# mvrl/RANGE

Measured on AMD Instinct MI355X. Metric: geo-embeddings/sec (10k-query batch, range_db_large), higher is better.
Workload: dtype f32

## Files before the change

range_amd/csrc/forward_host.h:

```cpp
#pragma once

struct ModelParams { float tau_sem, tau_geo, beta; };

static int model_params(const range_ctx* c, int32_t model, float beta, ModelParams& m) {
    if (model != RANGE_MODEL_RANGE && model != RANGE_MODEL_RANGE_PLUS)
        return fail(RANGE_ERR_INVALID, "unknown model %d", model);
    m.tau_sem = model == RANGE_MODEL_RANGE ? 15.0f : 12.0f;
    m.tau_geo = model == RANGE_MODEL_RANGE ? 0.0f : 40.0f;
    if (c->tau_sem_set > 0.f) m.tau_sem = c->tau_sem_set;
    if (c->tau_geo_set > 0.f && model == RANGE_MODEL_RANGE_PLUS) m.tau_geo = c->tau_geo_set;
    m.beta = model == RANGE_MODEL_RANGE ? 1.0f : beta;
    if (!(m.beta >= 0.f && m.beta <= 1.f)) return fail(RANGE_ERR_INVALID, "beta must be in [0,1]");
    return RANGE_OK;
}

static int forward_head(const range_ctx* c, const double* lonlat, const double* out, int32_t model, float beta, ModelParams& m) {
    if (!c || !lonlat || !out) return fail(RANGE_ERR_INVALID, "null argument");
    return model_params(c, model, beta, m);
}

static int forward_small(range_ctx* c, int64_t B, const ModelParams& m, double* out, hipStream_t s) {
    SmallArgs a{};
    int rc = softmax_scales(c, B, m.tau_sem, m.tau_geo, RANGE_MAX_TAU, a.k_sem, a.k_geo);
    if (rc) return rc;
    const SmallPlan p = plan_forward_small(c->n_cu, c->bank.n_rows, B, PLAN_CONSTS);
    HIP_TRY(c->pass.ws_small_o.ensure(p.o_floats));
    HIP_TRY(c->pass.ws_small_z.ensure(p.z_floats));
    a.keys = c->bank.d_keys.p;
    a.xyz4 = c->bank.d_xyz4.p;
    a.values = c->bank.d_values.p;
    a.ehat = c->pass.ws_ehat32.p;
    a.xq = c->pass.ws_xq.p;
    a.osum = c->pass.ws_small_o.p;
    a.zsum = c->pass.ws_small_z.p;
    a.B = B;
    a.n_valid = c->bank.n_rows;
    a.n_blocks = p.n_blocks;
    const bool geo = m.tau_geo > 0.f;
    static void (*const small_kernels[2][2])(SmallArgs) = {{attend_small_kernel<true, 2>, attend_small_kernel<true, 1>},
                                                          {attend_small_kernel<false, 2>, attend_small_kernel<false, 1>}};
    {
        ProfScope ps(c, RANGE_PROF_ATTEND, s);
        if (int lrc = launch(small_kernels[!geo][p.nq == 1], dim3((unsigned)p.n_wg), dim3(256), as_lds_bytes(p.nq), s, a)) return lrc;
    }
    rc = launch(small_finalize_kernel, dim3((unsigned)B, 8), dim3(1024), 0, s, c->pass.ws_small_o.p, c->pass.ws_small_z.p,
                p.n_wg, p.qcap, geo ? 1 : 0, geo ? m.beta : 1.0f, c->pass.ws_ehat64.p, out);
    if (rc) return rc;
    c->pass.last_qtiles = 1;
    c->pass.last_splits = p.n_wg;
    return RANGE_OK;
}

static int scan_workspace(range_ctx* c, int64_t B, const ModelParams& m, bool* kept, range_stream_t stream) {
    const int rc = range_scan_stats(c, c->pass.ws_ehat32.p, c->pass.ws_xq.p, B, m.tau_sem, m.tau_geo, c->pass.ws_stats.p, 0,
                                    nullptr, nullptr, 1, stream);
    *kept = c->kept.kept_B == B;
    return rc;
}

static int attend_workspace(range_ctx* c, int64_t p0, int64_t p1, const ModelParams& m, bool kept, SlabMap* map,
                            range_stream_t stream) {
    return attend_impl(c, c->pass.ws_ehat32.p + p0 * 256, c->pass.ws_xq.p + p0 * 4, p1 - p0, m.tau_sem, m.tau_geo, m.beta,
                       c->pass.ws_stats.p + p0 * 4, nullptr, map, kept ? p0 : -1, stream);
}

static int forward_chunked(range_ctx* c, int64_t B, const ModelParams& m, const FwdChunkPlan& plan, double* out,
                           range_stream_t stream, bool* chunked) {
    *chunked = false;
    ENTER_DEVICE(c);
    hipStream_t s = (hipStream_t)stream;
    const size_t n_chunks = plan.tiles.size();
    if (!c->ovl.aux_stream) {
        HIP_TRY(hipStreamCreateWithFlags(&c->ovl.aux_stream, hipStreamNonBlocking));
    }
    while (c->ovl.events.size() < n_chunks) {
        hipEvent_t e = nullptr;
        HIP_TRY(hipEventCreateWithFlags(&e, hipEventDisableTiming));
        c->ovl.events.push_back(e);
    }
    int64_t most_tiles = 0;
    for (int t : plan.tiles) most_tiles = std::max<int64_t>(most_tiles, t);
    HIP_TRY(c->pass.ws_stats_parts.ensure((size_t)plan.p1_splits * B * 4));
    HIP_TRY(c->pass.ws_slabs.ensure((size_t)plan.p2_splits * std::min<int64_t>(B, most_tiles * QTILE) * VAL_DIM));
    const float* ehat = c->pass.ws_ehat32.p;
    const float* xq = c->pass.ws_xq.p;
    float* stats = c->pass.ws_stats.p;
    std::vector<int64_t> cuts{0};
    for (int t : plan.tiles) cuts.push_back(std::min<int64_t>(B, cuts.back() + (int64_t)t * QTILE));
    if (int rc = scan_stats_impl(c, ehat, xq, cuts[1], m.tau_sem, m.tau_geo, stats, 0, nullptr, nullptr, 1, 0, B,
                                 plan.p1_splits, stream))
        return rc;
    if (c->kept.kept_B != cuts[1]) return RANGE_OK;
    *chunked = true;
    HIP_TRY(hipEventRecord(c->ovl.events[0], s));
    HIP_TRY(hipStreamWaitEvent(c->ovl.aux_stream, c->ovl.events[0], 0));
    size_t recorded = 0;
    auto joined = [&](int rc) {
        (void)hipStreamWaitEvent(s, c->ovl.events[recorded], 0);
        return rc;
    };
    for (size_t i = 1; i < n_chunks; ++i) {
        const int64_t q0 = cuts[i], nq = cuts[i + 1] - q0;
        if (int rc = scan_stats_impl(c, ehat + q0 * KEY_DIM, xq + q0 * 4, nq, m.tau_sem, m.tau_geo, stats + q0 * 4, 0, nullptr, nullptr,
                                     1, q0, B, plan.p1_splits, (range_stream_t)c->ovl.aux_stream, true,
                                     (size_t)plan.p1_splits * q0 * 4))
            return joined(rc);
        HIP_TRY(hipEventRecord(c->ovl.events[i], c->ovl.aux_stream));
        recorded = i;
    }
    for (size_t i = 0; i < n_chunks; ++i) {
        const int64_t q0 = cuts[i], nq = cuts[i + 1] - q0;
        if (i > 0) HIP_TRY(hipStreamWaitEvent(s, c->ovl.events[i], 0));
        SlabMap map{};
        if (int rc = attend_impl(c, ehat + q0 * KEY_DIM, xq + q0 * 4, nq, m.tau_sem, m.tau_geo, m.beta, stats + q0 * 4, nullptr, &map, q0,
                                 stream, nullptr, 0, plan.p2_splits))
            return joined(rc);
        HIP_TRY(launch_finalize(c->pass.ws_slabs.p, map, c->pass.ws_ehat64.p + q0 * KEY_DIM, nq, 0, nq, out + q0 * RANGE_OUT_DIM, s));
    }
    c->pass.last_qtiles = (int)((B + QTILE - 1) / QTILE);
    c->pass.last_splits = plan.p2_splits;
    return RANGE_OK;
}

extern "C" {

int range_forward(range_ctx* c, const double* lonlat, int64_t B, int32_t model, float beta,
                  double* out, range_stream_t stream) {
    ModelParams m;
    if (int rc = forward_head(c, lonlat, out, model, beta, m)) return rc;
    c->pass.ws_queries = 0;
    if (int rc = encode_to_workspace(c, lonlat, B, nullptr, stream)) return rc;
    if (plan_temperatures(m.tau_sem, m.tau_geo, B, c->sw.small_forward).one_pass) {
        c->pass.ws_queries = B;
        ENTER_DEVICE(c);
        return forward_small(c, B, m, out, (hipStream_t)stream);
    }
    if (c->sw.allow_keep && c->bank.pv_mode == RANGE_PV_EXACT && c->bank.has_bank &&
        plan_temperatures(m.tau_sem, m.tau_geo, B, false).shift == SHIFT_CONSTANT) {
        const FwdChunkPlan plan = plan_forward_chunks(c->n_cu, plan_pass1(c->n_cu, c->bank.n_rows, B, false, 0, PLAN_CONSTS),
                                                      plan_pass2(c->n_cu, c->bank.n_rows, B, c->sw.p2_streamk, PLAN_CONSTS),
                                                      c->sw.fwd_overlap);
        if (plan.tiles.size() >= 2) {
            bool chunked = false;
            if (int rc = forward_chunked(c, B, m, plan, out, stream, &chunked)) return rc;
            if (chunked) {
                c->pass.ws_queries = B;
                return RANGE_OK;
            }
        }
    }
    bool kept = false;
    SlabMap map{};
    if (int rc = scan_workspace(c, B, m, &kept, stream)) return rc;
    if (int rc = attend_workspace(c, 0, B, m, kept, &map, stream)) return rc;
    c->pass.ws_queries = B;
    ENTER_DEVICE(c);
    HIP_TRY(launch_finalize(c->pass.ws_slabs.p, map, c->pass.ws_ehat64.p, B, 0, B, out, (hipStream_t)stream));
    return RANGE_OK;
}

int range_host_copy(range_ctx* c, void* dst, const void* src, size_t bytes) {
    if (!c || !dst || !src) return fail(RANGE_ERR_INVALID, "null argument");
    if (!c->host.pool) c->host.pool.reset(new HostCopyPool(HostCopyPool::default_threads()));
    c->host.pool->copy(dst, src, bytes);
    return RANGE_OK;
}

int range_forward_host(range_ctx* c, const double* lonlat, int64_t B, int32_t model, float beta,
                       double* out_host, range_stream_t stream) {
    ModelParams m;
    if (int rc0 = forward_head(c, lonlat, out_host, model, beta, m)) return rc0;
    if (B <= 0) return fail(RANGE_ERR_INVALID, "B must be > 0");
    ENTER_DEVICE(c);
    hipStream_t s = (hipStream_t)stream;
    const size_t row_bytes = (size_t)RANGE_OUT_DIM * sizeof(double);
    HIP_TRY(c->host.ws_out64.ensure((size_t)B * RANGE_OUT_DIM));
    if (c->host.h_stage_bytes < (size_t)B * row_bytes) {
        if (c->host.h_stage) (void)hipHostFree(c->host.h_stage);
        c->host.h_stage = nullptr;
        c->host.h_stage_bytes = 0;
        HIP_TRY(hipHostMalloc(&c->host.h_stage, (size_t)B * row_bytes, hipHostMallocDefault));
        c->host.h_stage_bytes = (size_t)B * row_bytes;
    }
    if (!c->host.copy_stream) HIP_TRY(hipStreamCreateWithFlags(&c->host.copy_stream, hipStreamNonBlocking));
    if (!c->host.pool) c->host.pool.reset(new HostCopyPool(HostCopyPool::default_threads()));

    c->pass.ws_queries = 0;
    int rc = encode_to_workspace(c, lonlat, B, nullptr, stream);
    if (rc) return rc;
    c->pass.ws_queries = B;
    if (plan_temperatures(m.tau_sem, m.tau_geo, B, c->sw.small_forward).one_pass) {
        rc = forward_small(c, B, m, c->host.ws_out64.p, s);
        if (rc) return rc;
        HIP_TRY(hipMemcpyAsync(c->host.h_stage, c->host.ws_out64.p, (size_t)B * row_bytes, hipMemcpyDeviceToHost, s));
        HIP_TRY(hipStreamSynchronize(s));
        if (int rc2 = check_async_error(c)) return rc2;
        std::memcpy(out_host, c->host.h_stage, (size_t)B * row_bytes);
        return RANGE_OK;
    }
    bool kept = false;
    rc = scan_workspace(c, B, m, &kept, stream);
    if (rc) return rc;

    std::vector<int64_t> cuts{0, B};
// ... 54 lines not shown
```

range_amd/csrc/host_plan.h:

```cpp
#pragma once
#include <algorithm>
#include <cmath>
#include <cstddef>
#include <cstdint>
#include <vector>

namespace range_host {

inline int choose_splits(int n_qtiles, int n_blocks, int n_cu, int wg_per_cu, int max_splits,
                         double split_cost = 0.002) {
    const double slots = (double)n_cu * wg_per_cu;
    const int cap = std::max(1, std::min(max_splits, n_blocks / 4));
    const int ns_min = std::min(cap, (int)std::ceil(slots / n_qtiles));
    int best = ns_min;
    double best_score = -1e9;
    for (int ns = ns_min; ns <= cap; ++ns) {
        const double total = (double)n_qtiles * ns;
        const double rounds = std::ceil(total / slots);
        double score = total / (rounds * slots);
        if (rounds < 4) score *= 0.85 + 0.0375 * rounds;
        score -= split_cost * (ns - ns_min);
        if (score > best_score) { best_score = score; best = ns; }
        if (ns - ns_min > 64) break;
    }
// ... 284 lines not shown
    size_t part_floats = 0;
    int64_t topk_slots = 0;
    int topk_chunks = 0;
};

inline Pass1Plan plan_pass1(int n_cu, int64_t n_rows, int64_t B, bool topk_scan, int force_splits, const PlanConsts& K) {
    Pass1Plan p;
    p.n_blocks = (int32_t)((n_rows + K.blk - 1) / K.blk);
    p.n_qtiles = (int32_t)((B + K.qtile - 1) / K.qtile);
    const bool few = B <= 4 * K.qtile;
    p.n_splits = choose_splits(p.n_qtiles, p.n_blocks, n_cu, K.p1_wg_per_cu,
                               topk_scan ? (few ? 256 : 16) : (few ? 2048 : 128));
    if (force_splits > 0) p.n_splits = std::max(1, std::min<int>(force_splits, std::max(1, p.n_blocks / 4)));
    p.grid = p.n_splits * p.n_qtiles;
    p.merge_by_wave = p.n_splits > 32;
    p.part_floats = (size_t)p.n_splits * B * 4;
    p.topk_slots = (B + 15) / 16;
    p.topk_chunks = (int)std::max<int64_t>(1, std::min<int64_t>(
        std::min<int64_t>(64, p.n_blocks / 32 > 0 ? p.n_blocks / 32 : 1),
        ((int64_t)16 * n_cu + p.topk_slots - 1) / p.topk_slots));
    return p;
}

struct KeptStatsPlan {
    int n_qtiles = 0, n_blocks = 0, n_splits = 0;
    int grid = 0;
    bool merge_by_wave = false;
    struct Group { int first, count; };
    std::vector<Group> groups;
    size_t part_floats = 0;
    size_t ws_floats = 0;
};

inline ShiftMode kept_pair_shift(float tau_sem, float tau_geo) { return plan_temperatures(tau_sem, tau_geo, 0, false).shift; }

inline KeptStatsPlan plan_kept_stats(int n_cu, int64_t n_rows, int64_t B, int n_pairs, int force_splits, int max_pairs,
                                     const PlanConsts& K) {
    KeptStatsPlan p;
    const Pass1Plan s = plan_pass1(n_cu, n_rows, B, false, force_splits, K);
    p.n_qtiles = s.n_qtiles;
    p.n_blocks = s.n_blocks;
    p.n_splits = s.n_splits;
    p.grid = s.grid;
    p.merge_by_wave = s.merge_by_wave;
    p.part_floats = s.part_floats;
    for (int first = 0; first < n_pairs; first += max_pairs)
        p.groups.push_back({first, std::min(max_pairs, n_pairs - first)});
    p.ws_floats = p.part_floats * (size_t)std::min(max_pairs, std::max(n_pairs, 0));
    return p;
}

struct Pass2Plan {
    int n_qtiles = 0, n_blocks = 0;
    int n_splits = 0;
    bool streamk = false;
    int sk_cols = 1, sk_groups = 0;
    int grid = 0;
    size_t slab_floats = 0;
};

inline Pass2Plan plan_pass2(int n_cu, int64_t n_rows, int64_t B, bool allow_streamk, const PlanConsts& K,
                            int force_splits = 0) {
    Pass2Plan p;
    p.n_blocks = (int32_t)((n_rows + K.blk - 1) / K.blk);
    p.n_qtiles = (int32_t)((B + K.qtile - 1) / K.qtile);
    p.n_splits = choose_splits(p.n_qtiles, p.n_blocks, n_cu, 1,
                               std::max(32, std::min(512, (n_cu + p.n_qtiles - 1) / p.n_qtiles)),
                               std::max(0.001, 140.0 / (double)n_rows));
    if (force_splits > 0) p.n_splits = std::max(1, std::min<int>(force_splits, std::max(1, p.n_blocks / 4)));
    constexpr int P2_STREAMK_ROWS = 50000;
    p.streamk = allow_streamk && n_rows <= P2_STREAMK_ROWS;
    if (p.streamk) {
        constexpr int P2_COL_ROWS = 16384;
        p.sk_cols = (int32_t)std::max<int64_t>(1, std::min<int64_t>((n_rows + P2_COL_ROWS - 1) / P2_COL_ROWS,
                                                                    std::max(1, p.n_blocks / 4)));
        const int64_t Uc = (int64_t)p.n_qtiles * (p.n_blocks / p.sk_cols);
        p.sk_groups = (int32_t)std::max<int64_t>(1, std::min<int64_t>(n_cu, Uc / 4));
        p.slab_floats = (size_t)p.sk_cols * (p.sk_groups + p.n_qtiles) * K.qtile * K.val_dim;
    } else {
        p.slab_floats = (size_t)p.n_splits * B * K.val_dim;
    }
    p.grid = p.streamk ? p.sk_groups : p.n_splits * p.n_qtiles;
    return p;
}

struct FwdChunkPlan {
    std::vector<int> tiles;
    int p1_splits = 0, p2_splits = 0;
};

constexpr int FWD_CHUNK_FILL_PCT = 98;
inline FwdChunkPlan plan_forward_chunks(int n_cu, const Pass1Plan& p1, const Pass2Plan& p2, int overlap) {
    FwdChunkPlan p;
    p.p1_splits = p1.n_splits;
    p.p2_splits = p2.n_splits;
    const int T = p2.n_qtiles, ns = p2.n_splits;
    if (overlap == 0 || p2.streamk || T < 2 || ns < 1 || n_cu < 1) return p;
    if (overlap > 0) {
        for (int t0 = 0; t0 < T && overlap < T; t0 += overlap) p.tiles.push_back(std::min(overlap, T - t0));
        return p;
    }
    const int64_t R = ((int64_t)T * ns + n_cu - 1) / n_cu;
    for (int64_t C = std::min<int64_t>(R, T); C >= 2; --C) {
        std::vector<int> lo((size_t)C), hi((size_t)C);
        int64_t sum_lo = 0, sum_hi = 0;
        bool ok = true;
        for (int64_t i = 0; i < C && ok; ++i) {
            const int64_t r = R / C + (i >= C - R % C ? 1 : 0);
            const int64_t most = r * n_cu / ns;
            const int64_t fill = (FWD_CHUNK_FILL_PCT * r * n_cu + 100 * (int64_t)ns - 1) / (100 * (int64_t)ns);
            const int64_t least = std::max<int64_t>(std::max<int64_t>(fill, (r - 1) * n_cu / ns + 1), 1);
            ok = least <= most;
            lo[(size_t)i] = (int)least;
            hi[(size_t)i] = (int)most;
            sum_lo += least;
            sum_hi += most;
        }
        if (!ok || sum_lo > T || sum_hi < T) continue;
        p.tiles = hi;
        int64_t excess = sum_hi - T;
        for (size_t i = 0; i < p.tiles.size() && excess > 0; ++i) {
            const int64_t d = std::min<int64_t>(excess, hi[i] - lo[i]);
            p.tiles[i] -= (int)d;
            excess -= d;
        }
        return p;
    }
    return p;
}

struct TopkPlan {
    int n_groups = 0, n_blocks = 0;
    bool gemm = false;
    int G = 1;
    int n_wg = 0;
    bool fused = false;
    size_t cand_keys = 0, cand_dmax = 0;
    int key_e2 = 0;
    int n_qblocks = 0, n_splits = 0, grid = 0;
    int tile_stride = 1;
};

inline TopkPlan plan_topk(int n_cu, int64_t n_rows, int64_t B, float key_norm_max, bool topk_gemm, bool bf16,
                          bool topks_fused, bool force_exact, int tg_sample, const PlanConsts& K) {
    TopkPlan p;
    p.n_groups = (int)((B + 15) / 16);
    p.n_blocks = (int)((n_rows + K.blk - 1) / K.blk);
    constexpr int NWV = 4;
    p.G = p.n_groups <= 1 ? 1 : 2;
    p.n_wg = std::max(1, std::min(std::min(n_cu, 256), (p.n_blocks + NWV - 1) / NWV));
    p.fused = topks_fused && B <= p.n_wg;
    p.cand_keys = (size_t)p.n_groups * 16 * p.n_wg * K.topks_wl;
    p.cand_dmax = (size_t)p.n_groups * 16 * p.n_wg;
    (void)std::frexp((double)key_norm_max, &p.key_e2);
    const bool tg_bank_ok = key_norm_max > 0.f && std::isfinite(key_norm_max) && std::abs(14 - p.key_e2) <= 100;
    p.gemm = topk_gemm && bf16 && B > 256 && p.n_blocks >= 64 && !force_exact && B <= 60000 && tg_bank_ok;
    if (p.gemm) {
        p.n_qblocks = (int32_t)((B + K.tg_qblock - 1) / K.tg_qblock);
        p.n_splits = std::max(4, std::min(std::min(K.tg_wg_per_cu * n_cu / p.n_qblocks, p.n_blocks / 8), 64));
        p.grid = p.n_qblocks * p.n_splits;
        p.tile_stride = std::max(1, std::min(tg_sample, p.n_blocks / p.n_splits / 4));
    }
    return p;
}

struct SmallPlan {
// ... 744 lines not shown
```

range_amd/csrc/pass2.h:

```cpp
#pragma once
#include "scan_common.h"

namespace range_hip {

__device__ __forceinline__ unsigned long long stamp() {
    unsigned long long t;
    asm volatile("s_memtime %0\n\ts_waitcnt lgkmcnt(0)" : "=s"(t) :: "memory");
    return t;
}
#define RANGE_WAIT_BARRIER_DIAG(n, vm, bar)                                   \
    do {                                                                      \
        const unsigned long long t0_ = stamp();                               \
        asm volatile("s_waitcnt vmcnt(" #n ") lgkmcnt(0)" ::: "memory");      \
        const unsigned long long t1_ = stamp();                               \
        asm volatile("s_barrier" ::: "memory");                               \
        const unsigned long long t2_ = stamp();                               \
        vm += t1_ - t0_; bar += t2_ - t1_;                                    \
    } while (0)
#define RANGE_WB(n, vm, bar)                                                  \
    do { if (DIAG) RANGE_WAIT_BARRIER_DIAG(n, vm, bar); else RANGE_WAIT_BARRIER(n); } while (0)

struct PvCarry {
    f32x4 v0a, v1a, v0b, v1b;
    float w0, w1;
// ... 463 lines not shown
                            const int ii = h / 6;
                            if (ii == 0) {
                                dma_b128(ssrc2, vvoff, sdst);
                            } else if (ii == 1) {
                                dma_b32(xsrc2, (uint32_t)(lane << 2), xdst);
                            } else if (ii < 18) {
                                const int p = ii - 2, hh = p >> 3, row = (p >> 2) & 1, qq = p & 3;
                                if (qq == 0) dma_group_begin(vdst + hh * (VB_BYTES / 2) + row * 4096);
                                dma_b128_q(vsrc1 + (8 * hh + row) * VAL_DIM, vvoff, qq);
                            }
                        }
                    } else if (h >= 150 && h < 206 && (h & 1) == 0) {
                        const int k = (h - 150) >> 1, r = k / 7, op = k % 7;
                        if (op == 0) e1[r] = fmaf(sv[r], a.k_sem, -wc.m1);
                        else if (op == 1) { if (GEO) e2[r] = fmaf(cg[r], a.k_geo, -wc.m2); }
                        else if (op == 2) e1[r] = __builtin_amdgcn_exp2f(e1[r]);
                        else if (op == 3) { if (GEO) e2[r] = __builtin_amdgcn_exp2f(e2[r]); }
                        else if (op == 4) e1[r] = valu_mul(wc.ca, e1[r]);
                        else if (op == 5) { if (GEO) e1[r] = valu_fma(wc.cb, e2[r], e1[r]); }
                        else w_next[r] = e1[r];
                    }
                });
    };

    if (nb > 0) {
        const int valid_last = n_left - (nb - 1) * BLK;
        int t = 0;
        for (; t + 2 <= nb; t += 2) {
            run_block(IntC<0>{}, t, w_a, w_b);
            if (t + 2 == nb && valid_last < BLK) zero_pad_rows(w_b, prow, valid_last);
            run_block(IntC<1>{}, t + 1, w_b, w_a);
        }
        if (t < nb) {
            if (valid_last < BLK) zero_pad_rows(w_a, prow, valid_last);
            run_block(IntC<0>{}, t, w_a, w_b);
        }
        carry_wait_states();
        pv_exec_carry(acc, carry);
    }
    asm volatile("s_waitcnt vmcnt(0)" ::: "memory");

    store_acc_tile(acc, out_tile, qt, wave, lane, a.B);
    }
}


template <int UNROLL>
__device__ __forceinline__ f32x4 sum_parts(const float* parts, const SlabMap& m, int64_t B, int64_t q, int c4) {
    f32x4 s = {0.f, 0.f, 0.f, 0.f};
    for (int col = 0; col < slab_cols(m); ++col) {
        int64_t first4, stride4;
        int n;
        slab_parts(m, B, q, col, first4, stride4, n);
        const f32x4* p4 = reinterpret_cast<const f32x4*>(parts) + first4 + c4;
        if (col == 0) s = p4[0];
#pragma unroll UNROLL
        for (int p = col == 0 ? 1 : 0; p < n; ++p) s += p4[(int64_t)p * stride4];
    }
    return s;
}

__global__ void reduce_parts_kernel(const float* parts, SlabMap m, int64_t B, float* out) {
    const int64_t i = (int64_t)blockIdx.x * blockDim.x + threadIdx.x;
    if (i >= B * (VAL_DIM / 4)) return;
    const int64_t q = i / (VAL_DIM / 4);
    const int c4 = (int)(i - q * (VAL_DIM / 4));
    reinterpret_cast<f32x4*>(out)[i] = sum_parts<4>(parts, m, B, q, c4);
}

__global__ void blend_kernel(const float* G, const float* H, float beta, int64_t n4, float* out) {
    const int64_t i = (int64_t)blockIdx.x * blockDim.x + threadIdx.x;
    if (i >= n4) return;
    const f32x4 g = reinterpret_cast<const f32x4*>(G)[i];
    const f32x4 h = reinterpret_cast<const f32x4*>(H)[i];
    const float a = 1.0f - beta;
    f32x4 o;
#pragma unroll
    for (int k = 0; k < 4; ++k) o[k] = __fadd_rn(__fmul_rn(a, g[k]), __fmul_rn(beta, h[k]));
    reinterpret_cast<f32x4*>(out)[i] = o;
}

__global__ void finalize_kernel(const float* parts, SlabMap m, const double* ehat64, int64_t B,
                                int64_t q0, int64_t nq, double* out) {
    const int64_t i = (int64_t)blockIdx.x * blockDim.x + threadIdx.x;
    if (i >= nq * 320) return;
    const int64_t q = q0 + i / 320;
    const int c = (int)(i % 320);
    double* o = out + q * 1280 + 4 * c;
    if (c < 256) {
        const f32x4 s = sum_parts<8>(parts, m, B, q, c);
        o[0] = (double)s.x; o[1] = (double)s.y; o[2] = (double)s.z; o[3] = (double)s.w;
    } else {
        const double* e = ehat64 + q * 256 + 4 * (c - 256);
        o[0] = e[0]; o[1] = e[1]; o[2] = e[2]; o[3] = e[3];
    }
}

}
```

range_amd/csrc/scan_host.h:

```cpp
#pragma once

static_assert(MAX_TAU_CONSTANT == RANGE_MAX_TAU && MAX_TAU_SHARP == RANGE_MAX_TAU_SHARP, "host_plan.h and range_hip.h disagree");

static int softmax_scales(range_ctx* c, int64_t B, float tau_sem, float tau_geo, float max_tau, float& k_sem, float& k_geo) {
    if (!c->bank.has_bank) return fail(RANGE_ERR_STATE, "bank not set (range_set_bank)");
    if (!c->bank.has_values)
        return fail(RANGE_ERR_STATE, "keys-only bank (range_set_keys): only range_topk_stream runs on it");
    if (B <= 0) return fail(RANGE_ERR_INVALID, "B must be > 0");
    if (!plan_temperatures(tau_sem, tau_geo, B, false).valid)
        return fail(RANGE_ERR_INVALID, "temperatures must be finite, > 0 and at most %g (tau_sem %g, tau_geo %g; tau_geo <= 0: "
                    "no geographic head): beyond that the softmax is an argmax to float32 precision",
                    (double)RANGE_MAX_TAU_SHARP, (double)tau_sem, (double)tau_geo);
    if (!(c->bank.key_norm_max <= 1.001f))
        return fail(RANGE_ERR_INVALID, "bank keys are not L2-normalised or not finite (largest row norm %.4f): the softmax of "
                    "range_scan_stats / range_attend needs unit keys, as range/range.py:85-89 prepares them "
                    "(range_topk_stream accepts any norm)", (double)c->bank.key_norm_max);
    if (tau_geo > 0.f && !(c->bank.xyz_norm_max <= 1.001f))
        return fail(RANGE_ERR_INVALID, "bank locations are not unit vectors or not finite (largest row norm %.4f): the geographic "
                    "softmax needs them as range/utils/utils.py:11-16 computes them", (double)c->bank.xyz_norm_max);
    if (tau_sem > max_tau || tau_geo > max_tau)
        return fail(RANGE_ERR_INVALID, "internal: temperatures above %g reached a constant-shift kernel", (double)max_tau);
    const double LOG2E = 1.4426950408889634;
    k_sem = (float)(tau_sem * LOG2E);
    k_geo = tau_geo > 0.f ? (float)(tau_geo * LOG2E) : 0.f;
    return RANGE_OK;
}

static int fill_scan_args(range_ctx* c, ScanArgs& a, const float* ehat32, const float* xq, int64_t B,
                          float tau_sem, float tau_geo) {
    if (int rc = softmax_scales(c, B, tau_sem, tau_geo, RANGE_MAX_TAU_SHARP, a.k_sem, a.k_geo)) return rc;
    a.keys = c->bank.d_keys.p;
    a.xyz4 = c->bank.d_xyz4.p;
    a.values = c->bank.d_values.p;
    a.ehat = ehat32;
    a.xq = xq;
    a.B = B;
    a.n_valid = c->bank.n_rows;
    a.beta = 1.f;
    a.sk_cols = 1;
    return RANGE_OK;
}

static int launch_merge_stats(bool by_wave, const float* parts, int32_t n_parts, int64_t B, float* out, hipStream_t s) {
    const int per_wg = by_wave ? 4 : 256;
    return launch(by_wave ? merge_stats_wave_kernel : merge_stats_kernel, dim3((unsigned)((B + per_wg - 1) / per_wg)), dim3(256),
                  0, s, parts, n_parts, B, out);
}

static hipError_t launch_finalize(const float* slabs, const SlabMap& map, const double* ehat64, int64_t B, int64_t q0,
                                  int64_t nq, double* out, hipStream_t s) {
    const int64_t n = nq * 320;
    hipLaunchKernelGGL(finalize_kernel, dim3((unsigned)((n + 255) / 256)), dim3(256), 0, s, slabs, map, ehat64, B, q0, nq, out);
    return hipGetLastError();
}

static int scan_stats_impl(range_ctx* c, const float* ehat32, const float* xq32, int64_t B, float tau_sem,
                           float tau_geo, float* stats, int topk, float* topk_val, int64_t* topk_idx,
                           int32_t keep_logits, int64_t first_query, int64_t total_queries, int32_t force_splits,
                           range_stream_t stream, bool beside = false, size_t parts_offset = 0) {
    if (!c || !ehat32 || !xq32 || !stats) return fail(RANGE_ERR_INVALID, "null argument");
    if (topk < 0 || topk > MAX_TOPK) return fail(RANGE_ERR_INVALID, "topk must be in [0,%d]", MAX_TOPK);
    if (topk > 0 && (!topk_val || !topk_idx)) return fail(RANGE_ERR_INVALID, "topk outputs null");
    if (first_query < 0 || first_query % QTILE != 0)
        return fail(RANGE_ERR_INVALID, "first_query must be a non-negative multiple of %d", QTILE);
    if (B > 0 && first_query + B > total_queries)
        return fail(RANGE_ERR_INVALID, "queries [%lld, %lld) exceed the scan's %lld", (long long)first_query,
                    (long long)(first_query + B), (long long)total_queries);
    if (force_splits < 0) return fail(RANGE_ERR_INVALID, "n_splits must be >= 0");
    ENTER_DEVICE(c);
    ScanArgs a{};
    hipStream_t s = (hipStream_t)stream;
    const bool extends = first_query > 0 && c->kept.kept_B == first_query && c->kept.kept_total == total_queries;
    if (first_query > 0 && !extends) keep_logits = 0;
    if (!extends) c->kept.kept_B = 0;
    bool write_logits = c->sw.allow_keep && (topk > 0 ? B > 0 : keep_logits != 0);
    const int64_t n_qtiles = (total_queries + QTILE - 1) / QTILE, n_blocks = (c->bank.n_rows + BLK - 1) / BLK;
    const size_t need = (size_t)n_qtiles * n_blocks * 1024;
    if (write_logits && extends) {
        if (need > c->kept.ws_logits.n || c->kept.kept_blocks != n_blocks) { write_logits = false; c->kept.kept_B = 0; }
    } else if (write_logits && need > c->kept.ws_logits.n) {
        size_t free_b = 0, total_b = 0;
        HIP_TRY(hipMemGetInfo(&free_b, &total_b));
        if (need * sizeof(float) <= free_b / 2) {
            HIP_TRY(c->kept.ws_logits.ensure(need));
        } else {
            write_logits = false;
            if (!c->kept.warned_no_keep) {
                c->kept.warned_no_keep = true;
                std::fprintf(stderr, "librange_hip: the logits of %lld queries x %lld bank rows (%.1f GB) do not fit in "
                             "half of the free device memory (%.1f GB free): not kept, pass 2 recomputes them\n",
                             (long long)B, (long long)c->bank.n_rows, need * 4e-9, free_b * 1e-9);
            }
        }
    }
    const bool topk_from_kept = topk > 0 && write_logits;
    const bool topk_scan = topk > 0 && !topk_from_kept;
    int rc = fill_scan_args(c, a, ehat32, xq32, B, tau_sem, tau_geo);
    if (rc) return rc;
    const TempRoute route = plan_temperatures(tau_sem, tau_geo, B, c->sw.small_forward);
    if (topk_scan && !route.topk_scan_ok)
        return fail(RANGE_ERR_INVALID, "range_scan_stats(topk > 0) at a temperature above %g needs to keep its logits (this "
                    "context cannot: RANGE_KEEP_LOGITS=0 or not enough free memory): take the top-k from range_topk_stream",
                    (double)RANGE_MAX_TAU);
    const Pass1Plan p = plan_pass1(c->n_cu, c->bank.n_rows, B, topk_scan, force_splits, PLAN_CONSTS);
    a.n_blocks = p.n_blocks;
    a.n_qtiles = p.n_qtiles;
    a.n_splits = p.n_splits;
    if (write_logits) a.logits = c->kept.ws_logits.p;
    a.qt_offset = (int32_t)(first_query / QTILE);
    if (topk_from_kept) {
        HIP_TRY(c->kept.ws_rowmax.ensure(p.part_floats));
        HIP_TRY(c->kept.ws_theta.ensure((size_t)B));
        a.rowmax = c->kept.ws_rowmax.p;
    }
    HIP_TRY(c->pass.ws_stats_parts.ensure(parts_offset + p.part_floats));
    a.out = c->pass.ws_stats_parts.p + parts_offset;
    if (topk_scan) {
        HIP_TRY(c->topk.ws_cand_val.ensure(p.part_floats * MAX_TOPK));
        HIP_TRY(c->topk.ws_cand_idx.ensure(p.part_floats * MAX_TOPK));
        a.cand_val = c->topk.ws_cand_val.p;
        a.cand_idx = c->topk.ws_cand_idx.p;
    }
    const bool geo = tau_geo > 0.f;
    static void (*const scan_kernels[2][2])(ScanArgs) = {{scan_stats_kernel<true, true>, scan_stats_kernel<true, false>},
                                                        {scan_stats_kernel<false, true>, scan_stats_kernel<false, false>}};
    static void (*const sharp_kernels[2])(ScanArgs) = {sharp_scan_stats_kernel<true>, sharp_scan_stats_kernel<false>};
    static void (*const beside_kernels[2])(ScanArgs) = {scan_stats_beside_kernel<true>, scan_stats_beside_kernel<false>};
    if (beside && (topk > 0 || route.shift == SHIFT_RUNNING_MAX))
        return fail(RANGE_ERR_INVALID, "internal: pass 1 beside pass 2 has the constant shift and no top-k");
    {
        ProfScope ps(c, RANGE_PROF_SCAN_STATS, s);
        if (beside) {
            if (int lrc = launch(beside_kernels[!geo], dim3((unsigned)std::min(c->n_cu, p.grid)), dim3(256), BESIDE_LDS_BYTES, s, a)) return lrc;
        } else {
            void (*const kernel)(ScanArgs) = route.shift == SHIFT_RUNNING_MAX ? sharp_kernels[!geo] : scan_kernels[!geo][!topk_scan];
            if (int lrc = launch(kernel, dim3((unsigned)p.grid), dim3(256), SCAN_LDS_BYTES, s, a)) return lrc;
        }
    }
    if (a.logits && keep_logits) {
        c->kept.kept_B = first_query + B;
        c->kept.kept_total = total_queries;
        c->kept.kept_blocks = a.n_blocks;
    }
    rc = launch_merge_stats(p.merge_by_wave, a.out, a.n_splits, B, stats, s);
    if (rc) return rc;
    int n_parts = a.n_splits, per_part = 4 * MAX_TOPK;
    if (topk_from_kept) {
        const int n_chunks = p.topk_chunks;
        HIP_TRY(c->topk.ws_cand_val.ensure((size_t)n_chunks * B * MAX_TOPK));
        HIP_TRY(c->topk.ws_cand_idx.ensure((size_t)n_chunks * B * MAX_TOPK));
        rc = launch(topk_threshold_kernel, dim3((unsigned)((B + 3) / 4)), dim3(256), 0, s,
                    c->kept.ws_rowmax.p, a.n_splits, B, c->kept.ws_theta.p);
        if (rc) return rc;
        rc = launch(topk_from_logits_kernel, dim3((unsigned)((p.topk_slots + 3) / 4), (unsigned)n_chunks),
                    dim3(256), 0, s, c->kept.ws_logits.p, a.n_blocks, B, c->bank.n_rows, n_chunks,
                    c->kept.ws_theta.p, c->topk.ws_cand_val.p, c->topk.ws_cand_idx.p);
        if (rc) return rc;
        n_parts = n_chunks;
        per_part = MAX_TOPK;
    }
    if (topk <= 0) return RANGE_OK;
    return launch(merge_topk_wave_kernel, dim3((unsigned)((B + 3) / 4)), dim3(256), 0, s, c->topk.ws_cand_val.p,
                  c->topk.ws_cand_idx.p, n_parts, B, per_part, topk, c->bank.row_offset, topk_val, topk_idx);
}

static int attend_impl(range_ctx* c, const float* ehat32, const float* xq32, int64_t B, float tau_sem,
                       float tau_geo, float beta, const float* stats_global, float* partial,
                       SlabMap* map_out, int64_t kept_first, range_stream_t stream,
                       unsigned long long* diag_dev = nullptr, int64_t diag_capacity = 0, int32_t force_splits = 0) {
    if (!c || (!ehat32 && kept_first < 0) || !xq32 || !stats_global)
        return fail(RANGE_ERR_INVALID, "null argument");
    if (kept_first >= 0) {
        if (c->kept.kept_B <= 0) return fail(RANGE_ERR_STATE, "no kept logits (range_scan_stats with keep_logits)");
        if (kept_first % QTILE != 0) return fail(RANGE_ERR_INVALID, "first kept query must be a multiple of %d", QTILE);
        if (kept_first + B > c->kept.kept_B)
            return fail(RANGE_ERR_INVALID, "queries [%lld, %lld) exceed the %lld kept", (long long)kept_first,
                        (long long)(kept_first + B), (long long)c->kept.kept_B);
    }
    if (!diag_dev && !(beta >= 0.f && beta <= 1.f)) return fail(RANGE_ERR_INVALID, "beta must be in [0,1]");
    ENTER_DEVICE(c);
    ScanArgs a{};
    int rc = fill_scan_args(c, a, ehat32, xq32, B, tau_sem, tau_geo);
    if (rc) return rc;
    hipStream_t s = (hipStream_t)stream;
    const bool geo = tau_geo > 0.f;
    const bool bf16x3 = kept_first >= 0 && c->bank.pv_mode == RANGE_PV_BF16X3;
    if (bf16x3 && plan_temperatures(tau_sem, tau_geo, B, false).shift == SHIFT_RUNNING_MAX)
        return fail(RANGE_ERR_INVALID, "pv mode bf16x3 is not supported at temperatures above %g", (double)RANGE_MAX_TAU);
    const Pass2Plan p = plan_pass2(c->n_cu, c->bank.n_rows, B, c->sw.p2_streamk && !bf16x3 && !diag_dev, PLAN_CONSTS, force_splits);
    a.n_blocks = p.n_blocks;
    a.n_qtiles = p.n_qtiles;
    a.n_splits = p.n_splits;
    a.sk_cols = p.sk_cols;
    a.sk_groups = p.sk_groups;
    c->pass.last_qtiles = p.n_qtiles;
    c->pass.last_splits = p.streamk ? p.sk_groups : p.n_splits;
    if (diag_dev) {
        if (!geo) return fail(RANGE_ERR_INVALID, "diagnostic build exists for the geo variant only");
        if ((int64_t)p.grid * 4 * 16 > diag_capacity) return fail(RANGE_ERR_INVALID, "diag buffer too small");
    }
    HIP_TRY(c->pass.ws_slabs.ensure(p.slab_floats));
    const SlabMap map{a.n_splits, a.sk_groups, a.n_blocks, a.n_qtiles, a.sk_cols};
    a.out = c->pass.ws_slabs.p;
    a.stats = stats_global;
    a.beta = geo ? beta : 1.f;
    const dim3 grid((unsigned)p.grid), block(256);
    static void (*const bf16x3_kernels[2])(ScanArgs, const char*, int32_t) = {attend_bf16x3_kernel<true>,
                                                                             attend_bf16x3_kernel<false>};
    static void (*const stored_kernels[2])(ScanArgs) = {attend_stored_kernel<true>, attend_stored_kernel<false>};
    static void (*const recompute_kernels[2])(ScanArgs) = {attend_kernel<true>, attend_kernel<false>};
    if (diag_dev) {
        a.diag = diag_dev;
        return launch(attend_kernel<true, true>, grid, block, ATTEND_LDS_BYTES, s, a);
    }
    if (kept_first >= 0) {
        if (a.n_blocks != c->kept.kept_blocks) return fail(RANGE_ERR_STATE, "bank changed since the logits were kept");
        a.logits = c->kept.ws_logits.p;
        a.qt_offset = (int32_t)(kept_first / QTILE);
        ProfScope ps(c, RANGE_PROF_ATTEND, s);
        if (bf16x3) {
            const int32_t n_groups = (a.n_blocks + 1) / 2;
            if (c->bank.vplanes_groups != n_groups) return fail(RANGE_ERR_STATE, "bf16 planes of the values are missing");
            const char* planes = reinterpret_cast<const char*>(c->bank.d_vplanes.p);
            rc = launch(bf16x3_kernels[!geo], grid, block, PVB2_LDS_BYTES, s, a, planes, n_groups);
        } else {
            rc = launch(stored_kernels[!geo], grid, block, ATTEND_STORED_LDS_BYTES, s, a);
        }
    } else {
        ProfScope ps(c, RANGE_PROF_ATTEND, s);
        rc = launch(recompute_kernels[!geo], grid, block, ATTEND_LDS_BYTES, s, a);
    }
    if (rc) return rc;
    if (map_out) *map_out = map;
    if (partial) {
        const int64_t total4 = B * (VAL_DIM / 4);
        return launch(reduce_parts_kernel, dim3((unsigned)((total4 + 255) / 256)), dim3(256), 0, s,
                      c->pass.ws_slabs.p, map, B, partial);
    }
    return RANGE_OK;
}

extern "C" {

int range_scan_stats(range_ctx* c, const float* ehat32, const float* xq32, int64_t B, float tau_sem,
                     float tau_geo, float* stats, int topk, float* topk_val, int64_t* topk_idx,
                     int32_t keep_logits, range_stream_t stream) {
    return scan_stats_impl(c, ehat32, xq32, B, tau_sem, tau_geo, stats, topk, topk_val, topk_idx, keep_logits,
                           0, B, 0, stream);
}

int range_scan_stats_at(range_ctx* c, const float* ehat32, const float* xq32, int64_t B, float tau_sem,
                        float tau_geo, float* stats, int64_t first_query, int64_t total_queries,
                        int32_t n_splits, range_stream_t stream) {
    return scan_stats_impl(c, ehat32, xq32, B, tau_sem, tau_geo, stats, 0, nullptr, nullptr, 1,
                           first_query, total_queries, n_splits, stream);
}

int32_t range_p1_splits(const range_ctx* c, int64_t B) {
    if (!c || !c->bank.has_bank || B <= 0) return 0;
    return plan_pass1(c->n_cu, c->bank.n_rows, B, false, 0, PLAN_CONSTS).n_splits;
}

int64_t range_kept_queries(const range_ctx* c) { return c ? c->kept.kept_B : 0; }

int range_stats_kept(range_ctx* c, int64_t first_query, const float* xq32, int64_t B, int32_t n_taus,
                     const float* taus_sem, const float* taus_geo, int32_t n_splits, float* stats,
                     range_stream_t stream) {
    if (!c || !xq32 || !taus_sem || !taus_geo || !stats) return fail(RANGE_ERR_INVALID, "null argument");
    if (n_taus < 1) return fail(RANGE_ERR_INVALID, "n_taus must be >= 1");
    if (n_splits < 0) return fail(RANGE_ERR_INVALID, "n_splits must be >= 0");
    if (c->kept.kept_B <= 0) return fail(RANGE_ERR_STATE, "no kept logits (range_scan_stats with keep_logits)");
    if (first_query < 0 || first_query % QTILE != 0)
        return fail(RANGE_ERR_INVALID, "first kept query must be a non-negative multiple of %d", QTILE);
    if (B <= 0) return fail(RANGE_ERR_INVALID, "B must be > 0");
    if (first_query + B > c->kept.kept_B)
        return fail(RANGE_ERR_INVALID, "queries [%lld, %lld) exceed the %lld kept", (long long)first_query,
                    (long long)(first_query + B), (long long)c->kept.kept_B);
    ENTER_DEVICE(c);
    hipStream_t s = (hipStream_t)stream;
    const KeptStatsPlan p = plan_kept_stats(c->n_cu, c->bank.n_rows, B, n_taus, n_splits, KEPT_MAX_PAIRS, PLAN_CONSTS);
    KeptStatsArgs a{};
    std::vector<float> k_sem((size_t)n_taus), k_geo((size_t)n_taus);
    for (int i = 0; i < n_taus; ++i)
        if (int rc = softmax_scales(c, B, taus_sem[i], taus_geo[i], RANGE_MAX_TAU_SHARP, k_sem[i], k_geo[i])) return rc;
    if (p.n_blocks != c->kept.kept_blocks) return fail(RANGE_ERR_STATE, "bank changed since the logits were kept");
    HIP_TRY(c->kept.ws_stat_parts.ensure(p.ws_floats));
    a.logits = c->kept.ws_logits.p;
    a.xyz4 = c->bank.d_xyz4.p;
    a.xq = xq32;
    a.out = c->kept.ws_stat_parts.p;
    a.B = B;
    a.n_valid = c->bank.n_rows;
    a.n_blocks = p.n_blocks;
    a.n_qtiles = p.n_qtiles;
    a.n_splits = p.n_splits;
    a.qt_offset = (int32_t)(first_query / QTILE);
    static void (*const kept_kernels[KEPT_MAX_PAIRS][2])(KeptStatsArgs) = {
        {kept_stats_kernel<1, true>, kept_stats_kernel<1, false>}, {kept_stats_kernel<2, true>, kept_stats_kernel<2, false>},
        {kept_stats_kernel<3, true>, kept_stats_kernel<3, false>}, {kept_stats_kernel<4, true>, kept_stats_kernel<4, false>},
        {kept_stats_kernel<5, true>, kept_stats_kernel<5, false>}, {kept_stats_kernel<6, true>, kept_stats_kernel<6, false>},
        {kept_stats_kernel<7, true>, kept_stats_kernel<7, false>}, {kept_stats_kernel<8, true>, kept_stats_kernel<8, false>}};
    for (const KeptStatsPlan::Group& grp : p.groups) {
        a.sharp_mask = a.geo_mask = 0u;
        for (int i = 0; i < grp.count; ++i) {
            const float ts = taus_sem[grp.first + i], tg = taus_geo[grp.first + i];
            a.k_sem[i] = k_sem[grp.first + i];
            a.k_geo[i] = k_geo[grp.first + i];
            if (kept_pair_shift(ts, tg) == SHIFT_RUNNING_MAX) a.sharp_mask |= 1u << i;
            if (tg > 0.f) a.geo_mask |= 1u << i;
        }
        {
            ProfScope ps(c, RANGE_PROF_KEPT_STATS, s);
            if (int rc = launch(kept_kernels[grp.count - 1][a.geo_mask == 0u], dim3((unsigned)p.grid), dim3(256), 0, s, a)) return rc;
        }
        for (int i = 0; i < grp.count; ++i)
            if (int rc = launch_merge_stats(p.merge_by_wave, c->kept.ws_stat_parts.p + (size_t)i * p.part_floats, p.n_splits, B,
                                            stats + (size_t)(grp.first + i) * B * 4, s))
                return rc;
    }
    return RANGE_OK;
// ... 72 lines not shown
```

Before: 533,800.

## Run chunk finalize on the auxiliary stream with per-chunk slab regions

Each chunk's attention now writes partial slabs into its own region of a larger slab buffer, so the finalize for chunk i no longer has to finish before chunk i+1's attention. All finalizes except the last run on the auxiliary stream. They are capped to a small grid via a grid-stride loop, which leaves most CUs free for the next attention kernel. The auxiliary stream is joined back at the end. The cost is a bigger slab workspace (with a fallback to the old layout if allocation fails) and possible contention between finalize and attend.

Measured after the change: 534,700, median of 6. Within noise of the previous version (+0.2%).

```diff
diff --git a/range_amd/csrc/forward_host.h b/range_amd/csrc/forward_host.h
--- a/range_amd/csrc/forward_host.h
+++ b/range_amd/csrc/forward_host.h
@@ -64,6 +64,8 @@
                        c->pass.ws_stats.p + p0 * 4, nullptr, map, kept ? p0 : -1, stream);
 }
 
+constexpr int FIN_BESIDE_CUS_PER_WG = 4;
+
 static int forward_chunked(range_ctx* c, int64_t B, const ModelParams& m, const FwdChunkPlan& plan, double* out,
                            range_stream_t stream, bool* chunked) {
     *chunked = false;
@@ -73,15 +75,20 @@
     if (!c->ovl.aux_stream) {
         HIP_TRY(hipStreamCreateWithFlags(&c->ovl.aux_stream, hipStreamNonBlocking));
     }
-    while (c->ovl.events.size() < n_chunks) {
+    while (c->ovl.events.size() < 2 * n_chunks) {
         hipEvent_t e = nullptr;
         HIP_TRY(hipEventCreateWithFlags(&e, hipEventDisableTiming));
         c->ovl.events.push_back(e);
     }
+    const hipEvent_t aux_end = c->ovl.events[2 * n_chunks - 1];
     int64_t most_tiles = 0;
     for (int t : plan.tiles) most_tiles = std::max<int64_t>(most_tiles, t);
     HIP_TRY(c->pass.ws_stats_parts.ensure((size_t)plan.p1_splits * B * 4));
-    HIP_TRY(c->pass.ws_slabs.ensure((size_t)plan.p2_splits * std::min<int64_t>(B, most_tiles * QTILE) * VAL_DIM));
+    const bool regions = c->pass.ws_slabs.ensure(slab_region_floats(plan.p2_splits, B, PLAN_CONSTS)) == hipSuccess;
+    if (!regions) {
+        (void)hipGetLastError();
+        HIP_TRY(c->pass.ws_slabs.ensure((size_t)plan.p2_splits * std::min<int64_t>(B, most_tiles * QTILE) * VAL_DIM));
+    }
     const float* ehat = c->pass.ws_ehat32.p;
     const float* xq = c->pass.ws_xq.p;
     float* stats = c->pass.ws_stats.p;
@@ -94,10 +101,15 @@
     *chunked = true;
     HIP_TRY(hipEventRecord(c->ovl.events[0], s));
     HIP_TRY(hipStreamWaitEvent(c->ovl.aux_stream, c->ovl.events[0], 0));
-    size_t recorded = 0;
     auto joined = [&](int rc) {
-        (void)hipStreamWaitEvent(s, c->ovl.events[recorded], 0);
+        const hipError_t e = hipEventRecord(aux_end, c->ovl.aux_stream);
+        const hipError_t w = e == hipSuccess ? hipStreamWaitEvent(s, aux_end, 0) : e;
+        if (rc == RANGE_OK && w != hipSuccess)
+            return fail(RANGE_ERR_HIP, "forward in chunks: joining the auxiliary stream failed: %s", hipGetErrorString(w));
         return rc;
+    };
+    auto hip_joined = [&](hipError_t e, const char* what) {
+        return e == hipSuccess ? RANGE_OK : joined(fail(RANGE_ERR_HIP, "%s failed: %s", what, hipGetErrorString(e)));
     };
     for (size_t i = 1; i < n_chunks; ++i) {
         const int64_t q0 = cuts[i], nq = cuts[i + 1] - q0;
@@ -105,21 +117,32 @@
                                      1, q0, B, plan.p1_splits, (range_stream_t)c->ovl.aux_stream, true,
                                      (size_t)plan.p1_splits * q0 * 4))
             return joined(rc);
-        HIP_TRY(hipEventRecord(c->ovl.events[i], c->ovl.aux_stream));
-        recorded = i;
+        if (int rc = hip_joined(hipEventRecord(c->ovl.events[i], c->ovl.aux_stream), "hipEventRecord")) return rc;
     }
     for (size_t i = 0; i < n_chunks; ++i) {
         const int64_t q0 = cuts[i], nq = cuts[i + 1] - q0;
-        if (i > 0) HIP_TRY(hipStreamWaitEvent(s, c->ovl.events[i], 0));
+        if (i > 0)
+            if (int rc = hip_joined(hipStreamWaitEvent(s, c->ovl.events[i], 0), "hipStreamWaitEvent")) return rc;
         SlabMap map{};
         if (int rc = attend_impl(c, ehat + q0 * KEY_DIM, xq + q0 * 4, nq, m.tau_sem, m.tau_geo, m.beta, stats + q0 * 4, nullptr, &map, q0,
-                                 stream, nullptr, 0, plan.p2_splits))
+                                 stream, nullptr, 0, plan.p2_splits, regions ? q0 : 0))
             return joined(rc);
-        HIP_TRY(launch_finalize(c->pass.ws_slabs.p, map, c->pass.ws_ehat64.p + q0 * KEY_DIM, nq, 0, nq, out + q0 * RANGE_OUT_DIM, s));
+        const bool deferred = regions && i + 1 < n_chunks;
+        hipStream_t fs = deferred ? c->ovl.aux_stream : s;
+        if (deferred) {
+            const hipEvent_t attended = c->ovl.events[n_chunks + i];
+            if (int rc = hip_joined(hipEventRecord(attended, s), "hipEventRecord")) return rc;
+            if (int rc = hip_joined(hipStreamWaitEvent(fs, attended, 0), "hipStreamWaitEvent")) return rc;
+        }
+        const float* slabs = c->pass.ws_slabs.p + (regions ? slab_region_floats(map.n_parts, q0, PLAN_CONSTS) : 0);
+        if (int rc = hip_joined(launch_finalize(slabs, map, c->pass.ws_ehat64.p + q0 * KEY_DIM, nq, 0, nq, out + q0 * RANGE_OUT_DIM, fs,
+                                                deferred ? std::max<int64_t>(1, c->n_cu / FIN_BESIDE_CUS_PER_WG) : 0),
+                                "finalize_kernel"))
+            return rc;
     }
     c->pass.last_qtiles = (int)((B + QTILE - 1) / QTILE);
     c->pass.last_splits = plan.p2_splits;
-    return RANGE_OK;
+    return regions ? joined(RANGE_OK) : RANGE_OK;
 }
 
 extern "C" {
diff --git a/range_amd/csrc/host_plan.h b/range_amd/csrc/host_plan.h
--- a/range_amd/csrc/host_plan.h
+++ b/range_amd/csrc/host_plan.h
@@ -390,6 +390,10 @@
     }
     p.grid = p.streamk ? p.sk_groups : p.n_splits * p.n_qtiles;
     return p;
+}
+
+inline size_t slab_region_floats(int n_splits, int64_t q0, const PlanConsts& K) {
+    return (size_t)n_splits * (size_t)q0 * (size_t)K.val_dim;
 }
 
 struct FwdChunkPlan {
diff --git a/range_amd/csrc/pass2.h b/range_amd/csrc/pass2.h
--- a/range_amd/csrc/pass2.h
+++ b/range_amd/csrc/pass2.h
@@ -569,18 +569,19 @@
 
 __global__ void finalize_kernel(const float* parts, SlabMap m, const double* ehat64, int64_t B,
                                 int64_t q0, int64_t nq, double* out) {
-    const int64_t i = (int64_t)blockIdx.x * blockDim.x + threadIdx.x;
-    if (i >= nq * 320) return;
-    const int64_t q = q0 + i / 320;
-    const int c = (int)(i % 320);
-    double* o = out + q * 1280 + 4 * c;
-    if (c < 256) {
-        const f32x4 s = sum_parts<8>(parts, m, B, q, c);
-        o[0] = (double)s.x; o[1] = (double)s.y; o[2] = (double)s.z; o[3] = (double)s.w;
-    } else {
-        const double* e = ehat64 + q * 256 + 4 * (c - 256);
-        o[0] = e[0]; o[1] = e[1]; o[2] = e[2]; o[3] = e[3];
-    }
-}
-
-}
+    const int64_t stride = (int64_t)gridDim.x * blockDim.x;
+    for (int64_t i = (int64_t)blockIdx.x * blockDim.x + threadIdx.x; i < nq * 320; i += stride) {
+        const int64_t q = q0 + i / 320;
+        const int c = (int)(i % 320);
+        double* o = out + q * 1280 + 4 * c;
+        if (c < 256) {
+            const f32x4 s = sum_parts<8>(parts, m, B, q, c);
+            o[0] = (double)s.x; o[1] = (double)s.y; o[2] = (double)s.z; o[3] = (double)s.w;
+        } else {
+            const double* e = ehat64 + q * 256 + 4 * (c - 256);
+            o[0] = e[0]; o[1] = e[1]; o[2] = e[2]; o[3] = e[3];
+        }
+    }
+}
+
+}
diff --git a/range_amd/csrc/scan_host.h b/range_amd/csrc/scan_host.h
--- a/range_amd/csrc/scan_host.h
+++ b/range_amd/csrc/scan_host.h
@@ -48,9 +48,11 @@
 }
 
 static hipError_t launch_finalize(const float* slabs, const SlabMap& map, const double* ehat64, int64_t B, int64_t q0,
-                                  int64_t nq, double* out, hipStream_t s) {
+                                  int64_t nq, double* out, hipStream_t s, int64_t most_wgs = 0) {
     const int64_t n = nq * 320;
-    hipLaunchKernelGGL(finalize_kernel, dim3((unsigned)((n + 255) / 256)), dim3(256), 0, s, slabs, map, ehat64, B, q0, nq, out);
+    int64_t wgs = (n + 255) / 256;
+    if (most_wgs > 0) wgs = std::min(wgs, most_wgs);
+    hipLaunchKernelGGL(finalize_kernel, dim3((unsigned)wgs), dim3(256), 0, s, slabs, map, ehat64, B, q0, nq, out);
     return hipGetLastError();
 }
 
@@ -167,7 +169,8 @@
 static int attend_impl(range_ctx* c, const float* ehat32, const float* xq32, int64_t B, float tau_sem,
                        float tau_geo, float beta, const float* stats_global, float* partial,
                        SlabMap* map_out, int64_t kept_first, range_stream_t stream,
-                       unsigned long long* diag_dev = nullptr, int64_t diag_capacity = 0, int32_t force_splits = 0) {
+                       unsigned long long* diag_dev = nullptr, int64_t diag_capacity = 0, int32_t force_splits = 0,
+                       int64_t slab_first_query = 0) {
     if (!c || (!ehat32 && kept_first < 0) || !xq32 || !stats_global)
         return fail(RANGE_ERR_INVALID, "null argument");
     if (kept_first >= 0) {
@@ -199,9 +202,12 @@
         if (!geo) return fail(RANGE_ERR_INVALID, "diagnostic build exists for the geo variant only");
         if ((int64_t)p.grid * 4 * 16 > diag_capacity) return fail(RANGE_ERR_INVALID, "diag buffer too small");
     }
-    HIP_TRY(c->pass.ws_slabs.ensure(p.slab_floats));
+    const size_t slab_off = slab_region_floats(p.n_splits, slab_first_query, PLAN_CONSTS);
+    if (slab_first_query < 0 || (slab_first_query > 0 && (p.streamk || slab_off + p.slab_floats > c->pass.ws_slabs.n)))
+        return fail(RANGE_ERR_INVALID, "internal: the slab region of query %lld does not exist", (long long)slab_first_query);
+    HIP_TRY(c->pass.ws_slabs.ensure(slab_off + p.slab_floats));
     const SlabMap map{a.n_splits, a.sk_groups, a.n_blocks, a.n_qtiles, a.sk_cols};
-    a.out = c->pass.ws_slabs.p;
+    a.out = c->pass.ws_slabs.p + slab_off;
     a.stats = stats_global;
     a.beta = geo ? beta : 1.f;
     const dim3 grid((unsigned)p.grid), block(256);
@@ -235,7 +241,7 @@
     if (partial) {
         const int64_t total4 = B * (VAL_DIM / 4);
         return launch(reduce_parts_kernel, dim3((unsigned)((total4 + 255) / 256)), dim3(256), 0, s,
-                      c->pass.ws_slabs.p, map, B, partial);
+                      a.out, map, B, partial);
     }
     return RANGE_OK;
 }
```
